# ckonst/VNDecorrelate

Hardware: AMD Instinct MI355X
Metric: Msamples/sec decorrelated (stereo, 30 taps) + achieved HBM GB/s vs roofline (higher is better)
Workload: dtype f32

## Files before the change

### vndecorrelate_amd/csrc/vnd_hooks.hpp

```cpp
#pragma once

extern "C" {

vnd_status vnd_time_convolve_f32_dev(vnd_ctx *ctx, const vnd_taps *t, const float *x, float *y, int64_t batch,
                                     int64_t n, int32_t C, int32_t mode, int32_t n_buffers, int64_t stride,
                                     int32_t iters, void *stream_, float *avg_ms)
{
    vnd_status st = check_shape(ctx, t, batch, n, C, mode);
    if (st != VND_OK) return st;
    if (!avg_ms || iters <= 0 || n_buffers <= 0) return fail(VND_ERR_INVALID, "bad timing arguments");
    DeviceScope on(ctx->device);
    hipStream_t stream = (hipStream_t)stream_;
    hipEvent_t e0 = nullptr, e1 = nullptr;
    hipError_t he = hipEventCreate(&e0);
    if (he == hipSuccess) he = hipEventCreate(&e1);
    if (he == hipSuccess) he = hipEventRecord(e0, stream);
    for (int i = 0; he == hipSuccess && st == VND_OK && i < iters; ++i) {
        const int64_t off = (int64_t)(i % n_buffers) * stride;
        st = launch(ctx, t, x + off, y + off, batch, n, C, mode, stream);
    }
    float ms = 0.f;
    if (he == hipSuccess) he = hipEventRecord(e1, stream);
    if (he == hipSuccess) he = hipEventSynchronize(e1);
    if (he == hipSuccess) he = hipEventElapsedTime(&ms, e0, e1);
// ... 93 lines not shown

vnd_status vnd_spec_kernel_source(int32_t C, const int32_t *tap_offsets, const int32_t *tap_index,
                                  const float *tap_weight, int32_t mode, char *text, int64_t capacity, int64_t *bytes)
{
    if (mode != VND_MODE_FAST && mode != VND_MODE_EXACT)
        return fail(VND_ERR_INVALID, "the specialised kernel exists for VND_MODE_FAST and VND_MODE_EXACT");
    if (!bytes) return fail(VND_ERR_INVALID, "null bytes pointer");
    const Tuning tun = tuning_snapshot();
    SpecTable t;
    if (vnd_status st = spec_table_from_csr(C, tap_offsets, tap_index, tap_weight, nullptr, nullptr, nullptr, 0, &t); st != VND_OK) return st;
    SpecConfig cfg;
    if (!spec_pick_config(t, tun, 160 * 1024, 0, 0, &cfg, false, false, mode == VND_MODE_EXACT)) return fail(VND_ERR_UNSUPPORTED, "halo does not fit the LDS ring");
    cfg.exact = mode == VND_MODE_EXACT ? 1 : 0;
    return source_out(spec_prologue(t, cfg) + kSpecKernelSource, text, capacity, bytes);
}

vnd_status vnd_window_kernel_source(int32_t C, const int32_t *tap_offsets, const int32_t *tap_index,
                                    const float *tap_weight, const int32_t *seg_offsets, const int32_t *seg_end,
                                    const float *seg_gain, int32_t apply_gain, int32_t mode, int32_t frames_per_lane,
                                    int32_t threads, char *text, int64_t capacity, int64_t *bytes,
                                    int64_t *lds_bytes_per_tile, int64_t *fmas_per_tile)
{
    if (mode != VND_MODE_FAST && mode != VND_MODE_EXACT)
        return fail(VND_ERR_INVALID, "the specialised kernel exists for VND_MODE_FAST and VND_MODE_EXACT");
    if (!bytes) return fail(VND_ERR_INVALID, "null bytes pointer");
    const Tuning tun = tuning_snapshot();
    SpecTable t;
    if (vnd_status st = spec_table_from_csr(C, tap_offsets, tap_index, tap_weight, seg_offsets, seg_end, seg_gain, apply_gain, &t); st != VND_OK)
        return st;
    const int M = frames_per_lane, G = tun.win_g > 0 ? tun.win_g : 8;
    WinGeom g;
    bool quad = C % 8 == 0 && tun.win_quad != 0 && tun.win_octet != 0 && win_geometry(t, M, threads, G, false, 160 * 1024, &g, 2);
    quad = quad || ((C % 4 == 0 || (C % 4 == 2 && C >= 6)) && tun.win_quad != 0 && win_geometry(t, M, threads, G, false, 160 * 1024, &g, 1));
    const bool split = !quad && C == 2 && tun.win_split > 0 && win_geometry(t, M, threads, G, false, 160 * 1024, &g, 0, true);
    const bool bc = C == 2 && tun.win_source_fanout != 0;
    if (bc && !win_geometry(t, M, threads, G, true, 160 * 1024, &g, 0, split))
        return fail(VND_ERR_UNSUPPORTED, "this window geometry does not fit the LDS");
    if (!bc && !quad && !split && !win_geometry(t, M, threads, G, false, 160 * 1024, &g))
        return fail(VND_ERR_UNSUPPORTED, "this window geometry does not fit the LDS");
    SpecConfig cfg = win_config(t, g, tun, mode == VND_MODE_EXACT, bc);
    cfg.epi = (tun.win_source_epi != 0 && !bc && !split && (C == 2 || quad)) ? 1 : 0;
    if (lds_bytes_per_tile || fmas_per_tile) {
        size_t lb = 0, fm = 0;
        if (cfg.exact) win_traffic_exact(t, M, &lb, &fm);
        else win_traffic(t, M, &lb, &fm);
        if (lds_bytes_per_tile) *lds_bytes_per_tile = (int64_t)lb;
        if (fmas_per_tile) *fmas_per_tile = (int64_t)fm;
    }
    return source_out(win_source(t, g, cfg), text, capacity, bytes);
}

vnd_status vnd_code_object_private_bytes(const void *code, int64_t bytes, const char *kernel, int64_t *private_bytes)
{
    if (!code || bytes <= 0 || !kernel || !private_bytes) return fail(VND_ERR_INVALID, "bad arguments");
    const std::vector<char> image((const char *)code, (const char *)code + bytes);
    *private_bytes = spec_private_bytes(image, kernel);
    return VND_OK;
}

vnd_status vnd_tuning_read(const char *name, int32_t fallback, int32_t *value)
{
    if (!name || !value) return fail(VND_ERR_INVALID, "null name or value pointer");
    for (const TuningName &v : kTuningNames)
        if (strcmp(v.name, name) == 0) { *value = tuning_value(v, fallback); return VND_OK; }
    *value = fallback;
    return fail(VND_ERR_INVALID, "'%.64s' is not a registered tuning variable (kTuningNames, csrc/vnd_spec.hpp)", name);
}

vnd_status vnd_set_variant(vnd_ctx *ctx, int32_t variant)
// ... 125 lines not shown
```

### vndecorrelate_amd/csrc/vnd_spec.hpp

```cpp
#pragma once
#include <hip/hip_runtime.h>
#include <hip/hiprtc.h>
#include <stdint.h>

#include <sys/stat.h>
#include <sys/types.h>
#include <unistd.h>

#include <algorithm>
#include <cstdarg>
#include <cstring>
#include <cstdio>
#include <cstdlib>
#include <map>
#include <mutex>
#include <string>
#include <tuple>
#include <vector>

namespace vnd {

static const char kSpecKernelSource[] =
#include "vnd_spec_kernel.inc"
    ;

struct SpecConfig {
    int nt = 256;
    int rr = 2;
    int pp = 4;
    int dd = 1;
    int la = 8;
    int nt_stores = 0;
    int exact = 0;
    int epi = 0;
    int bc = 0;
    int shift = 0;
    int win = 0, win_g = 0, win_lds = 0, win_per_cu = 0;
    int win_xpose = 0;
    int win_q = 0;
    int win_s = 0;
    int adds = 0;
    int win_merged = 0;
    int win_late = 0;
    int win_stamps = 0, win_stamp_phases = 0, win_stamp_wave = 0;
    int tile() const { return win ? (win_s ? nt / 2 : (win_q ? nt / (4 * win_q) : nt)) * win : 2 * nt * rr; }
    size_t lds_bytes() const
    {
        if (win) return (size_t)win_lds;
        const size_t pl = (size_t)pp * tile() + 2 * nt + (shift ? 2 : 0);
        return (bc ? 1 : 2) * (shift ? 2 : 1) * pl * 4 + (size_t)2 * (nt / 64) * rr * 2 * 4;
    }
    bool operator<(const SpecConfig &o) const
    {
        return std::tie(nt, rr, pp, dd, la, nt_stores, exact, epi, bc, shift, win, win_g, win_xpose, win_q, win_s, adds, win_merged, win_late,
                        win_stamps, win_stamp_phases, win_stamp_wave) <
               std::tie(o.nt, o.rr, o.pp, o.dd, o.la, o.nt_stores, o.exact, o.epi, o.bc, o.shift, o.win, o.win_g, o.win_xpose, o.win_q, o.win_s,
                        o.adds, o.win_merged, o.win_late, o.win_stamps, o.win_stamp_phases, o.win_stamp_wave);
    }
};

struct SpecTable {
    int C = 0;
    std::vector<int32_t> tap_off;
    std::vector<int32_t> idx;
    std::vector<float> w;
    int max_index = 0;
    std::vector<float> w_raw;
    bool has_seg = false, apply_gain = false;
    std::vector<int32_t> seg_off, seg_end;
    std::vector<float> seg_gain;
};

#define VND_TUNING_VARIABLES(X) \
     \
    X("VND_SPEC_NT", spec_nt, 0) X("VND_SPEC_RR", spec_rr, -1) X("VND_SPEC_DD", spec_dd, -1) X("VND_SPEC_LA", spec_la, -1) \
    X("VND_SPEC_SHIFT", spec_shift, 1) X("VND_WIN_M", win_m, 32) X("VND_WIN_G", win_g, 0) X("VND_WIN_QUAD_M", win_quad_m, 32) \
    X("VND_WIN_SPLIT_LATE", win_split_late, -1) X("VND_WIN_SPLIT_SMALL_NT", win_split_small_nt, 256) \
     \
    X("VND_WIN_EXACT", win_exact, 1) X("VND_WIN_SPLIT_CLASS", win_split_class, 1) X("VND_WIN_QUAD", win_quad, 1) \
    X("VND_WIN_OCTET", win_octet, 1) X("VND_WIN_WIDE", win_wide, 0) X("VND_WIN_SPLIT", win_split, -1) \
    X("VND_WIN_SPLIT_FANOUT", win_split_fanout, 1) X("VND_WIN_FANOUT_EPI", win_fanout_epi, 1) X("VND_WIN_XPOSE_PAIRS", win_xpose_pairs, 1) \
    X("VND_WIN_ADDS", win_adds, 1) X("VND_WIN_EXACT_MERGED", win_exact_merged, 1) \
    X("VND_WIN_SOURCE_FANOUT", win_source_fanout, 0) X("VND_WIN_SOURCE_EPI", win_source_epi, 0) \
    X("VND_EPI_BLOCK_SUMS", epi_block_sums, 1) X("VND_EPI_SUMS_ONLY", epi_sums_only, 1) X("VND_EPI_WIDE", epi_wide, 1) \
    X("VND_EPI_SEQ_SPLIT", epi_seq_split, 1) X("VND_EPI_PAR_COALESCED", epi_par_coalesced, 1) \
     \
    X("VND_WIN_CHUNKS", win_chunks, 1) X("VND_WIN_BALANCE", win_balance, 1) X("VND_WIN_CHUNK_LEN0", win_chunk_len0, 0) \
    X("VND_WIN_STAGGER_TICKS", win_stagger_ticks, 300) X("VND_WIN_PACE", win_pace, 1) X("VND_WIN_PACE_MIN_TILES", win_pace_min_tiles, 16) \
    X("VND_NT_MIN_MB", nt_min_mb, 64) X("VND_NO_NT", no_nt, 0) X("VND_FORCE_NT", force_nt, 0) \
     \
    X("VND_WIN_STAMPS", win_stamps, 0) X("VND_WIN_STAMP_PHASES", win_stamp_phases, 1) X("VND_WIN_STAMP_WAVE", win_stamp_wave, 0)

struct Tuning {
#define VND_TUNING_FIELD(name, field, fallback) int field = fallback;
    VND_TUNING_VARIABLES(VND_TUNING_FIELD)
#undef VND_TUNING_FIELD
};

struct TuningName { const char *name; int Tuning::*field; };
static const TuningName kTuningNames[] = {
#define VND_TUNING_NAME(name, field, fallback) {name, &Tuning::field},
    VND_TUNING_VARIABLES(VND_TUNING_NAME)
#undef VND_TUNING_NAME
};

inline bool spec_tuning()
{
    static const bool on = [] { const char *e = getenv("VND_TUNING"); return e && *e && *e != '0'; }();
    return on;
}
// ... 474 lines not shown
```

### vndecorrelate_amd/csrc/vnd_win.hpp

```cpp
#pragma once
#include "vnd_spec.hpp"
#include <cmath>
#include <functional>

namespace vnd {

static const char kWinKernelSource[] =
#include "vnd_win_kernel.inc"
    ;

struct WinGeom {
    int M = 0, nt = 0, G = 8;
    int C = 2;
    int DE = 0;
    int R = 0;
    int NB = 0;
    int plane = 0;
    int npl = 2;
    int tail = 0;
    int quad = 0;
    int split = 0;
    int nh() const { return split ? nt / 2 : (quad ? nt / (4 * quad) : nt); }
    int quad_pad() const { return quad == 2 ? 16 : 0; }
    size_t lds_bytes() const { return (size_t)(quad ? 2 * quad : 1) * (size_t)npl * (size_t)(M / 4) * (size_t)plane + (size_t)quad_pad(); }
    int tile() const { return nh() * M; }
};

inline int win_workgroups_per_cu(const WinGeom &g);

inline bool win_geometry(const SpecTable &t, int M, int nt, int G, bool bc, size_t lds_limit, WinGeom *g, int quad = 0, bool split = false)
{
    if (split && (t.C != 2 || quad || nt % 128 != 0)) return false;
    if (!(M == 16 || M == 32 || M == 64) || nt % 64 != 0 || nt < 64 || nt > 1024 || G < 1) return false;
    if (quad && (quad > 2 || (t.C % (4 * quad) != 0 && !(quad == 1 && t.C % 4 == 2 && t.C >= 6)) || bc || nt % (256 * quad) != 0 || M * quad > 64 || M > 32)) return false;
    if ((int64_t)t.idx.size() * M > 32768) return false;
    if (t.C < 2 || (t.C & 1) || (bc && t.C != 2)) return false;
    g->M = M; g->nt = nt; g->G = G; g->npl = 2; g->C = t.C; g->quad = quad; g->split = split ? 1 : 0;
    const int nh = g->nh();
    const int qc = M / 4;
    auto lay_out = [&](int de, int tail = 0) {
        g->DE = de;
        g->R = nh + g->DE - tail;
        g->tail = tail;
        g->NB = g->DE / G + 1;
        int units = g->R + G + tail;
        const bool swz = qc == 8;
        const int mod_rule = swz ? 4 : std::max(2, 16 / qc), res_rule = swz ? 2 : std::max(1, 8 / qc);
        while (units % mod_rule != res_rule) ++units;
        g->plane = units * 16;
        if ((size_t)(qc - 1) * g->plane + (size_t)G * 16 >= 65536) return false;
        if ((size_t)qc * g->plane >= 65536) return false;
        return g->lds_bytes() <= lds_limit;
    };
    const int de = (t.max_index + M - 1) / M;
    if (!lay_out(de)) return false;
    const int aligned = de + (16 - (nh + de) % 16) % 16;
    if (aligned != de) {
        const int before = win_workgroups_per_cu(*g);
        WinGeom plain = *g;
        if (!(lay_out(aligned) && win_workgroups_per_cu(*g) >= before)) {
            *g = plain;
            const int cut = (nh + de) % 16;
            if (quad && cut > 0 && nh + de - cut >= nh + G && cut <= (nt / 64) * (64 / (M * quad))) {
                if (!(lay_out(de, cut) && win_workgroups_per_cu(*g) >= before)) *g = plain;
            }
        }
    }
    return true;
}

inline int win_waves_per_simd_max(int M, bool split = false) { return split ? (M <= 32 ? 3 : 2) : (M <= 16 ? 3 : (M <= 32 ? 2 : 1)); }

inline int win_workgroups_per_cu(const WinGeom &g)
{
    const int by_lds = (int)std::min<size_t>(std::min<size_t>(16, 2048 / g.nt), (160 * 1024) / g.lds_bytes());
    const int by_regs = std::max(1, win_waves_per_simd_max(g.M, g.split != 0) * 4 / (g.nt / 64));
    return std::max(1, std::min(by_lds, by_regs));
}

struct WinOp { int kind, acc, half; float w; int tap; };
struct WinRead { int ch, o; std::vector<WinOp> ops; };

inline std::vector<WinRead> win_schedule(const SpecTable &t, int ch, int M)
{
    std::vector<std::pair<int, float>> taps;
    for (int32_t k = t.tap_off[ch]; k < t.tap_off[ch + 1]; ++k)
        if (t.w[k] != 0.0f) taps.push_back({t.idx[k], t.w[k]});
    std::stable_sort(taps.begin(), taps.end(), [](const std::pair<int, float> &a, const std::pair<int, float> &b) { return a.first < b.first; });
    std::vector<WinRead> out;
    if (taps.empty()) return out;
    const int o_last = ((taps.back().first + M - 1) / 4) * 4;
    for (int o = 0; o <= o_last; o += 4) {
        WinRead rd{ch, o, {}};
        for (const auto &tp : taps) {
            const int i = tp.first;
            for (int h = 0; h < 2; ++h) {
                const int j = o + 2 * h - i;
                if ((i & 1) == 0) {
// ... 12 lines not shown

inline void win_traffic(const SpecTable &t, int M, size_t *lds_bytes, size_t *fmas)
{
    *lds_bytes = 0; *fmas = 0;
    for (int ch = 0; ch < t.C; ++ch) {
        *lds_bytes += 16 * win_schedule(t, ch, M).size();
        for (int32_t k = t.tap_off[ch]; k < t.tap_off[ch + 1]; ++k) if (t.w[k] != 0.0f) *fmas += (size_t)M;
    }
}

inline std::string win_taps_name(int pg) { return pg == 0 ? std::string("vw_taps") : "vw_taps_" + std::to_string(pg); }

inline std::string win_taps_channel_name(int pg, int ch)
{
    return pg == 0 ? "vw_taps_c" + std::to_string(ch) : "vw_taps_" + std::to_string(pg) + "c" + std::to_string(ch);
}

inline std::string win_taps_dispatch(const SpecTable &t)
{
    std::string s = "template <int PG> __device__ __forceinline__ void vw_taps_of(vw_lchar *const (&b)[2][VW_NBT], float (&o0)[VW_M], float (&o1)[VW_M])\n{\n";
    for (int pg = 0; pg < t.C / 2; ++pg)
        spec_append(s, "    %sif constexpr (PG == %d) %s(b, o0, o1);\n", pg ? "else " : "", pg, win_taps_name(pg).c_str());
    s += "}\n#define VW_DISPATCH(pg) switch (pg) {";
    for (int pg = 0; pg < t.C / 2; ++pg) spec_append(s, " case %d: vw_span<%d>(a, lds, stream, t_first, ntiles, flags, pace); break;", pg, pg);
    s += " default: break; }\n";
    return s;
}

inline std::string win_rd(const WinGeom &g, int ch, int o)
{
    const int dE = o / g.M, rr = (o % g.M) / 4;
    const int first_tail = g.R - g.nh() + 1;
    char buf[96];
    if (g.tail > 0 && dE >= first_tail) snprintf(buf, sizeof buf, "VW_RD(b[%d][%d], %d)", ch, g.NB + (dE - first_tail), rr * g.plane);
    else { const int kb = dE / g.G; snprintf(buf, sizeof buf, "VW_RD(b[%d][%d], %d)", ch, kb, (dE - kb * g.G) * 16 + rr * g.plane); }
    return buf;
}

inline bool win_adds_ok(const SpecTable &t)
{
    std::vector<float> mags;
    for (size_t k = 0; k < t.w.size(); ++k) {
        const float m = std::fabs(t.w[k]);
        if (m == 0.0f) continue;
        if (!std::isfinite(m) || m < 1e-18f || m > 1e18f) return false;
        if (std::find(mags.begin(), mags.end(), m) == mags.end()) mags.push_back(m);
        if (mags.size() > 8) return false;
    }
    for (int ch = 0; ch < t.C; ++ch) {
        std::vector<std::pair<int, float>> taps;
        for (int32_t k = t.tap_off[ch]; k < t.tap_off[ch + 1]; ++k)
            if (t.w[k] != 0.0f) taps.push_back({t.idx[k], std::fabs(t.w[k])});
        std::stable_sort(taps.begin(), taps.end(), [](const std::pair<int, float> &a, const std::pair<int, float> &b) { return a.first < b.first; });
        int changes = 0;
        for (size_t k = 1; k < taps.size(); ++k) changes += taps[k].second != taps[k - 1].second;
        if (changes > 8) return false;
    }
    return !mags.empty();
}

inline float win_unit_ratio(float from, float to) { return (float)((double)from / (double)to); }

inline void win_emit_adds_op(std::string &s, const std::string &acc, const std::string &x, bool pair, float w, float *unit)
{
    const float mag = std::fabs(w);
    const char sign = std::signbit(w) ? '-' : '+';
    if (*unit == 0.0f) spec_append(s, "    %s = %s %c %s;\n", acc.c_str(), pair ? "Z2" : "0.0f", sign, x.c_str());
// ... 517 lines not shown
        src += "template <int QD> __device__ __forceinline__ void vw_taps_of_channel(int pc, vw_lchar *const (&b)[2][VW_NBT], float (&o)[VW_M])\n{\n";
        const int nq = (t.C + nch - 1) / nch;
        for (int qd = 0; qd < nq; ++qd) {
            const int pair0 = (t.C % nch != 0 && qd == nq - 1) ? (t.C - nch) / 2 : qd * nch / 2;
            spec_append(src, "    %sif constexpr (QD == %d) {\n        switch (pc) {\n", qd ? "else " : "", qd);
            for (int pc = 0; pc < nch; ++pc)
                spec_append(src, "        %s %s(b, o, o); break;\n", pc + 1 < nch ? ("case " + std::to_string(pc) + ":").c_str() : "default:",
                            win_taps_channel_name(pair0 + pc / 2, pc & 1).c_str());
            src += "        }\n    }\n";
        }
        src += "}\n#define VW_TAPS_OF_CHANNEL(pc) vw_taps_of_channel<QD>(pc, b, o);\n#define VW_DISPATCH(pg) switch (pg) {";
        for (int qd = 0; qd < nq; ++qd) spec_append(src, " case %d: vw_span_qc<%d>(a, lds, stream, t_first, ntiles, flags, pace); break;", qd, qd);
        src += " default: break; }\n";
    } else if (g.split) {
        for (int ch = 0; ch < 2; ++ch) src += c.exact ? win_taps_function_exact(t, g, c.la, 0, ch) : win_taps_function(t, g, c.la, 0, ch, c.adds != 0);
        src += "template <int PG> __device__ void vw_taps_of(vw_lchar *const (&b)[2][VW_NBT], float (&o0)[VW_M], float (&o1)[VW_M]);      // (vw_span: not instantiated)\n";
        src += "#define VW_DISPATCH(pg) vw_span_s(a, lds, stream, t_first, ntiles, flags, pace);\n";
    } else {
        const bool merged = c.bc && !c.exact;
        for (int pg = 0; pg < t.C / 2; ++pg) src += c.exact ? (c.win_merged ? win_taps_function_exact_merged(t, g, c.la, pg) : win_taps_function_exact(t, g, c.la, pg)) : (merged ? win_taps_function_merged(t, g, c.la, pg, c.adds != 0) : win_taps_function(t, g, c.la, pg, -1, c.adds != 0));
        src += win_taps_dispatch(t);
    }
    src += fixed.substr(at + marker.size());
    return src;
}

inline SpecConfig win_config(const SpecTable &t, const WinGeom &g, const Tuning &tun, bool exact, bool bc)
{
    SpecConfig c;
    const int M = g.M;
    const bool split = g.split != 0, quad = g.quad != 0;
    c.nt = g.nt; c.win = M; c.win_g = g.G; c.win_lds = (int)g.lds_bytes(); c.win_q = g.quad; c.win_s = g.split;
    c.win_per_cu = win_workgroups_per_cu(g);
    c.rr = 0; c.pp = 0; c.dd = 0;
    c.exact = exact ? 1 : 0; c.bc = bc ? 1 : 0;
    c.la = tun.spec_la >= 0 ? tun.spec_la : ((split && M >= 64) ? (exact ? 3 : 2) : (M >= 32 ? 4 : 6));
    c.win_xpose = (split || quad) ? 0 : (tun.win_xpose_pairs != 0 ? 1 : 0);
    c.adds = (!exact && tun.win_adds != 0 && win_adds_ok(t)) ? 1 : 0;
    c.win_merged = (bc && exact && !split && !quad && tun.win_exact_merged != 0 && win_exact_merged_ok(t)) ? 1 : 0;
    if (split) {
        const int late = M >= 64 ? ((exact && !t.has_seg) ? M / 8 : M / 4 - 1) : 0;
        c.win_late = std::min(std::max(tun.win_split_late >= 0 ? tun.win_split_late : late, 0), M / 4 - 1);
    }
    c.win_stamps = std::min(std::max(tun.win_stamps, 0), 4096);
    c.win_stamp_phases = tun.win_stamp_phases != 0 ? 1 : 0;
    c.win_stamp_wave = std::max(0, tun.win_stamp_wave);
    return c;
}

inline bool win_pick_config(const SpecTable &t, const Tuning &tun, size_t lds_limit, int M, bool small_tiles, bool bc, SpecConfig *out,
                            const std::function<bool(const SpecConfig &)> &rejected, int quad, bool split, bool exact)
{
    static const int kShapes[] = {512, 384, 256, 192, 128, 64};
    const int nt_env = tun.spec_nt, g_env = tun.win_g;
    int best_waves = 0;
    for (int k = 0; k < 6; ++k) {
        const int nt = nt_env > 0 ? nt_env : kShapes[k];
        if (nt_env <= 0 && nt > 256 && quad < 2 && !split) continue;
        if (nt_env <= 0 && nt == 384) continue;
        if (small_tiles && nt_env <= 0 && nt > (quad ? 256 * quad : (split ? tun.win_split_small_nt : 128))) continue;
        for (int G : {8, 4}) {
            if (g_env > 0) G = g_env;
            WinGeom g;
            if (win_geometry(t, M, nt, G, bc, lds_limit, &g, quad, split)) {
                const int waves = win_workgroups_per_cu(g) * (nt / 64);
                if (waves > best_waves) {
                    SpecConfig c = win_config(t, g, tun, exact, bc);
                    if (rejected && rejected(c)) {
                        if (!c.win_xpose) {
                            bool found = false;
                            if (split && M >= 64 && tun.spec_la < 0)
                                while (!found && c.la > 1) { c.la -= 1; found = !rejected(c); }
                            if (!found) continue;
                            best_waves = waves;
                            *out = c;
                            continue;
                        }
                        bool found = false;
                        if (c.la > 3 && tun.spec_la < 0) {
                            c.la -= 1;
                            found = !rejected(c);
                            if (!found) c.la += 1;
                        }
                        if (!found) {
                            c.win_xpose = 0;
                            if (rejected(c)) continue;
                        }
                    }
                    best_waves = waves;
                    *out = c;
                }
            }
            if (g_env > 0) break;
        }
        if (nt_env > 0) break;
    }
    return best_waves > 0;
}

inline std::string win_source_for(const SpecTable &t, const SpecConfig &cfg)
{
    WinGeom g;
    if (!win_geometry(t, cfg.win, cfg.nt, cfg.win_g, cfg.bc != 0, 160 * 1024, &g, cfg.win_q, cfg.win_s != 0)) return "#error window geometry does not fit\n";
    if ((int)g.lds_bytes() != cfg.win_lds) return "#error window geometry changed between the launch plan and the build\n";
    return win_source(t, g, cfg);
}

}
```

### vndecorrelate_amd/csrc/vnd_win_kernel.inc

```
R"VNDWIN(
// vnd_spec_kernel, WINDOW form - the per-table tap sum with a register window (gfx950, wave64).
//
// Compiled at run time with hipRTC (vnd_win.hpp) behind a generated prologue that defines
//   VW_NT   threads per workgroup                 VW_M   consecutive output frames a lane owns per tile (16 | 32 | 64)
//   VW_R    ring entries (one entry = the M frames of one lane's run): NT of the tile + VW_DE of halo
//   VW_G    entries mirrored behind the ring, = the reach of one base register
//   VW_NB   base registers per channel (VW_DE / VW_G + 1)
//   VW_PLANE  bytes between the LDS planes of consecutive 16-byte chunks of an entry
//   VW_LA   LDS reads kept in flight ahead of the FMAs
//   VW_C    interleaved channels of the signal (even): a workgroup takes ONE channel pair of a span, 8 bytes of
//           every VW_C*4-byte frame (VW_C = 2: the whole frame, 16-byte accesses)
//   VW_Q    1: the QUAD form for signals of 4k channels - a workgroup takes a channel QUAD of a span (16 bytes of every
//           frame), a wave computes ONE channel of it (tap functions vw_taps_<pair>c<channel>) and stages and stores whole
//           16-byte pieces for all four (vw_span_qc below)
//           2: the OCTET form for signals of 8k channels - two neighbouring quads (32 bytes of every frame: with 8 channels,
//           whole frames and whole cache lines) per workgroup, an eighth of its lanes per channel
//   VW_S    1: the SPLIT form of a stereo signal - half the workgroup's waves compute channel 0, the others channel 1 (the tap
//           functions vw_taps_c0 / vw_taps_c1): a lane carries one channel's accumulators, so three waves fit a SIMD's registers
//           where the plain form holds two (vw_span_s below)
// and the functions vw_taps(), vw_taps_1(), ... (at the marker below): the tap sum of ONE lane for each channel
// pair, fully unrolled, with vw_taps_of<PG>() to pick one and VW_DISPATCH(pg): the span loop vw_span<pg> of a run-time pair number.
//
// The reference's tap sum (decorrelation.py:649-658, :402-414) asks, per output sample, for one input sample
// per tap.  vnd_spec_kernel.inc reads each of them from LDS (one aligned ds_read_b64 per tap and output
// ... 62 lines not shown
    int epi_nblocks;
    int epi_rows_major;      // 1: [stream][block][x0 x1 y0 y1] instead - the rows epilogue_reduce_kernel adds up (the fused fast stage)
    // PACING of a CU's two co-resident workgroups (one round of persistent workgroups): the SIMDs issue the OLDER wave first, so the
    // workgroup publishes its count of finished tiles in its CU's slot pair and reads its partner's: the one BEHIND runs its next tile at
    // raised wave priority.  pace: [CU index][2] counters in device memory (never reset: a stale count only costs the first tile its bias)
    unsigned *pace;
};

struct VWPace { unsigned *mine; const unsigned *other; unsigned done; };

constexpr int VW_NW = VW_NT / 64;
constexpr int VW_QC = VW_M / 4;                 // 16-byte chunks per entry and channel
constexpr int VW_NH = VW_S ? VW_NT / 2 : VW_Q ? VW_NT / (4 * VW_Q) : VW_NT;  // lanes - and ring entries of a tile - per channel pair
constexpr int VW_T = VW_NH * VW_M;              // frames per tile
constexpr int VW_LPE = VW_Q ? VW_M * VW_Q : VW_M / 2;  // lanes of a 1 KB global access that fall into one entry (a lane moves a frame pair; VW_Q: one frame of four channels)
constexpr int VW_EPI_N = 64 / VW_LPE;           // entries per 1 KB global access
constexpr int VW_NI = VW_M / 2;                 // 1 KB global accesses per wave and tile
constexpr int VW_NPL = 2;                       // plane sets in LDS: one per output channel (the store phase transposes both channels' runs through them)
constexpr int VW_NXP = (VW_BC && !VW_S) ? 1 : 2; // ... of them holding INPUT: a mono input is staged once for both outputs (in the split form into both sets)
constexpr int VW_CH = VW_QC * VW_PLANE;         // byte offset of channel 1's planes
constexpr int VW_CX = VW_BC ? 1 : VW_C;         // interleaved INPUT channels
// channel pairs (VW_Q: quads or octets): one per workgroup and span.  4k + 2 channels (6, 10, ...) as QUADS: k full quads and one more that
// starts at channel C - 4 - it overlaps its neighbour in one channel pair, which both workgroups compute and write with the same bits
// (a frame's 16 bytes per access instead of the pair form's 8, for (k + 1) / (k + 1/2) of the arithmetic)
constexpr int VW_PAIRS = VW_Q ? (VW_C + 4 * VW_Q - 1) / (4 * VW_Q) : VW_C / 2;
constexpr int VW_PAIRB = 2 * VW_CH;             // VW_Q: byte offset of the second pair's plane sets
constexpr int VW_QUADB = 2 * VW_PAIRB + VW_QUADPAD; // octets: ... of the second QUAD's (shifted by 16 bytes: the two quads of a frame - neighbouring lanes of the 4-byte staging accesses - in different banks)
static_assert(VW_C >= 2 && VW_C % 2 == 0 && (VW_C == 2 || !VW_BC) && (VW_C == 2 || VW_Q || !VW_EPI), "whole channel pairs; fan-out and fused pointwise steps are stereo (quads / octets: the normaliser's sums only)");
static_assert(VW_Q == 0 || VW_Q == 1 || VW_Q == 2, "pairs, quads or octets");
static_assert(!VW_S || (VW_C == 2 && !VW_Q && !VW_EPI && VW_NT % 128 == 0 && VW_M >= 16), "split form: a stereo table, whole waves per channel");
static_assert(!VW_Q || ((VW_C % (4 * VW_Q) == 0 || (VW_Q == 1 && VW_C % 4 == 2 && VW_C >= 6)) && VW_NT % (256 * VW_Q) == 0 && VW_M * VW_Q <= 64 && VW_M <= 32), "quad / octet form: whole channel quads (4k + 2 channels: the last quad overlaps), whole waves per channel");
static_assert(VW_M == 16 || VW_M == 32 || VW_M == 64, "run length");
constexpr int VW_NBT = VW_NB + VW_TAIL;          // base registers per channel: the ring's, then one per entry offset that reaches into the tail
static_assert(VW_NT % 64 == 0 && VW_R >= VW_NH && VW_R + VW_TAIL == VW_NH + VW_DE && (VW_TAIL == 0 || (VW_Q && VW_R % 16 == 0)), "ring (+ tail) = tile + halo");
static_assert(VW_NB * VW_G > VW_DE, "bases cover the halo");
static_assert((VW_PLANE / 16) >= VW_R + VW_G + VW_TAIL, "plane stride: room for ring + mirror (+ tail)");
static_assert((VW_QC - 1) * VW_PLANE + VW_G * 16 < 65536 && VW_CH < 65536, "ds offset field is 16 bits");
static_assert((VW_Q ? 2 * VW_Q : 1) * VW_NPL * VW_QC * VW_PLANE + VW_QUADPAD <= 160 * 1024 && VW_QUADPAD % 16 == 0, "LDS");

// Raw buffer descriptor (stride 0): num_records = bytes left in the stream, so loads past the end of
// the stream return 0 (the reference's dropped terms, decorrelation.py:656-658) and stores past it
// are discarded.  Built from kernel arguments, blockIdx and the tile counter only: lives in SGPRs.
__device__ __forceinline__ v4i vw_rsrc(const void *base, long long bytes)
{
    const long long cap = 0x7fffffff;
    const unsigned long long addr = (unsigned long long)base;
    v4i r;
    r.x = (int)(unsigned)addr;
    r.y = (int)((unsigned)(addr >> 32) & 0xffffu);
    r.z = (int)(bytes < 0 ? 0 : (bytes > cap ? cap : bytes));
    r.w = 0x00020000;
    return r;
}

// blocks b and b + 8 share an XCD (and its L2): give one XCD consecutive logical ids, so that neighbouring
// spans (whose halos overlap) share an L2
__device__ __forceinline__ unsigned vw_xcd_remap(unsigned b, unsigned nwg)
{
    const unsigned q = nwg >> 3, r = nwg & 7u, xcd = b & 7u;
    const unsigned start = xcd < r ? xcd * (q + 1) : r * (q + 1) + (xcd - r) * q;
    return start + (b >> 3);
}

// (a mod R) for a < 2R, without a comparison: a - R wraps past 2^32 when a < R
__device__ __forceinline__ unsigned vw_wrap(unsigned a)
{
    const unsigned b = a - (unsigned)VW_R;
// ... 563 lines not shown
}
#endif

#if VW_S
// ---- the SPLIT form of a stereo signal: a wave computes ONE channel ---------------------------------------
// The plain form's lane carries both channels' work one after the other: E / P accumulators, the first channel's finished
// outputs and a tile of prefetched frames - ~240 registers, two waves per SIMD.  Here waves 0 .. NW/2-1 run channel 0's tap
// function (vw_taps_c0) on the tile's NT/2 entries and the other half channel 1's: per lane one channel's accumulators, half
// the prefetch - three waves per SIMD fit (two workgroups of 384 lanes per CU: 12 waves), on the same ring and the same
// 1 KB global accesses.  A frame's two channels now sit in two waves: outputs go as planar runs into the tile's dead
// entries, one barrier more, then each wave reads back and stores the 32 entries it also refills (as vw_span_qc).
template <int CH>
__device__ __forceinline__ void vw_taps_ch(vw_lchar *const (&b)[2][VW_NBT], float (&o)[VW_M])
{
    if constexpr (CH == 0) vw_taps_c0(b, o, o);
    else vw_taps_c1(b, o, o);
}

__device__ __forceinline__ void vw_span_s(const VWArgs &a, vw_lchar *lds, long long stream, int t_first, int ntiles, int flags, VWPace &pace)
{
    constexpr int NWH = VW_NW / 2;                                       // waves per channel
    constexpr int NI = VW_M / 4;                                         // 1 KB global STORES per wave and tile (64 frame pairs each)
    // VW_BC - a mono input fanned out: the one input channel is staged into BOTH plane sets (each output channel's waves read their own
    // copy with the tap functions of the stereo form unchanged), 16 bytes = 4 frames per lane and access: half as many input accesses,
    // each 256 frames = 256 / M ring entries (stereo: 128 frames)
    constexpr int NIN = VW_BC ? VW_M / 8 : VW_M / 4;                     // 1 KB global LOADS per wave and tile
    constexpr int EIN = VW_BC ? 256 / VW_M : VW_EPI_N;                   // ring entries per load
    constexpr int XB = VW_BC ? 4 : 8;                                    // input bytes per frame
    // the refill's frames: NE accesses are prefetched a tile ahead and held in registers through the tap phase, the other
    // LATE are loaded at the start of the store phase that consumes them (64-frame runs: the accumulators need the room)
    constexpr int LATE = VW_LATE < NIN ? VW_LATE : NIN - 1;
    constexpr int NE = NIN - LATE;
    static_assert(VW_LATE >= 0 && LATE < NIN, "late refill accesses");
    const int tid = threadIdx.x;
    const int ln = tid & 63;
    const int wv = __builtin_amdgcn_readfirstlane(tid >> 6);
    const int pc = wv >= NWH ? 1 : 0;                                    // the wave's channel
    const int wl = wv - pc * NWH;
    const int tl = wl * 64 + ln;                                         // the entry of a tile this LANE computes (in its channel)
    const int we = wl * 64 + pc * 32;                                    // the first of the 32 entries this WAVE stages and stores (both channels)
    const long long f0 = (long long)t_first * VW_T;
    const float *xs = a.x + (stream * a.n + f0) * (XB / 4);
    float *ys = a.y + (stream * a.n + f0) * 2;
    const long long bytes_left = (a.n - f0) * 8;                         // (of the output)
    const long long need = ((long long)ntiles * VW_T + (long long)VW_DE * VW_M) * XB;
    const long long bytes_need = need < (a.n - f0) * XB ? need : (a.n - f0) * XB;
#if VW_LANE_SWIZZLE
    const int lq = (ln & ~24) | ((ln & 8) << 1) | ((ln & 16) >> 1);      // (as vw_span: the 8-byte staging writes and read-backs touch every bank once)
#else
    const int lq = ln;
#endif
    const int lane_e = lq / VW_LPE;
    const int lane_at = ((lq % VW_LPE) >> 1) * VW_PLANE + (lq & 1) * 8;
    // ... and in a 1 KB LOAD: stereo as above; mono - 4 frames = one 16-byte chunk of entry ln / (M / 4), written to both plane sets
    const int in_e = VW_BC ? ln / (VW_M / 4) : lane_e;
    const int in_at = VW_BC ? (ln % (VW_M / 4)) * VW_PLANE : lane_at;
    const int in16 = VW_BC ? ln * 16 : lq * 16;                          // the lane's byte offset in a load
    auto stage = [&](vw_lchar *at, v4f v) {
        if constexpr (VW_BC) { *(vw_lv4f *)at = v; *(vw_lv4f *)(at + VW_CH) = v; }
        else vw_write_pair(at, v);
    };
#if VW_STAMPS && VW_STAMP_PHASES
    const bool vw_stamp_on = blockIdx.x < VW_STAMPS && (a.chunk_tiles > 0 || a.bal_total > 0 || (unsigned)(stream * a.spans + t_first / a.tiles_per_span) == vw_xcd_remap(blockIdx.x, a.nblocks));
    if (vw_stamp_on && threadIdx.x == 0) {
        unsigned hw, xcc;
        asm volatile("s_getreg_b32 %0, hwreg(HW_REG_HW_ID)" : "=s"(hw));
        asm volatile("s_getreg_b32 %0, hwreg(HW_REG_XCC_ID)" : "=s"(xcc));
        vw_stamps[blockIdx.x * 16 + 15] = (unsigned long long)hw | ((unsigned long long)xcc << 32);
    }
#endif
    VW_STAMP_DECL;
    VW_STAMP(0);

    {
        const v4i rx = vw_rsrc(xs, bytes_need);
        constexpr int NFILL = (VW_R + EIN - 1) / EIN;
        constexpr int PER = (NFILL + VW_NW - 1) / VW_NW;
        constexpr int BATCH = 8;
        for (int k0 = 0; k0 < PER; k0 += BATCH) {
            v4f w[BATCH];
#pragma unroll
            for (int kk = 0; kk < BATCH; ++kk) {
                const int i = wv + VW_NW * (k0 + kk);
                w[kk] = vw_load4(rx, i * 1024 + in16, 0, VW_LOAD_AUX);
            }
#pragma unroll
            for (int kk = 0; kk < BATCH; ++kk) {
                const int i = wv + VW_NW * (k0 + kk);
                const int e = i * EIN + in_e;
                if (k0 + kk < PER && e < VW_R) {
                    stage(lds + in_at + e * 16, w[kk]);
                    if (e < VW_G) stage(lds + in_at + (e + VW_R) * 16, w[kk]);
                }
            }
        }
    }
    v4f pre[NE];
    {
        const long long f = ((long long)VW_R + we) * VW_M;
        const v4i rx = vw_rsrc(xs + f * (XB / 4), bytes_need - f * XB);
#pragma unroll
        for (int m = 0; m < NE; ++m) pre[m] = vw_load4(rx, 1024 * m + in16, 0, VW_LOAD_AUX);
    }
    asm volatile("s_waitcnt lgkmcnt(0)\n\ts_barrier" ::: "memory");
    VW_STAMP(1);
    bool hi = (flags & 2) != 0;                                          // (wave-uniform) raised priority: a chunk's first workgroup - or, paced, the one behind
    if (hi) __builtin_amdgcn_s_setprio(2);

    unsigned p0 = 0;
    for (int t = 0; t < ntiles; ++t) {
        // the last tile of the workgroup's last unit refills nothing: no loads, no staging writes, no barrier behind its stores
        const bool fin = (flags & 1) != 0 && t == ntiles - 1;
        const unsigned pw = vw_wrap(p0 + (unsigned)we);
        const unsigned pl = vw_wrap(p0 + (unsigned)tl);
        // (a lane's byte offset in a 1 KB access and its entry in it, made opaque per tile: hipcc otherwise hoists the sums with
        //  64-frame runs is what spilled)
        int lq16 = lq * 16, in16o = in16;
        unsigned pwl = pw + (unsigned)lane_e, pwi = pw + (unsigned)in_e;
        asm volatile("" : "+v"(lq16), "+v"(pwl));
        if constexpr (VW_BC) asm volatile("" : "+v"(in16o), "+v"(pwi));
        float o[VW_M];
        {
            vw_lchar *b[2][VW_NBT];
#pragma unroll
            for (int k = 0; k < VW_NB; ++k) {
                b[0][k] = lds + vw_wrap(pl + (unsigned)(k * VW_G)) * 16u;
                b[1][k] = b[0][k] + VW_CH;
            }
            if (pc == 0) vw_taps_ch<0>(b, o);
            else vw_taps_ch<1>(b, o);
        }
#pragma unroll
        for (int j = 0; j < VW_M; ++j) asm volatile("" : "+v"(o[j]));
        VW_STAMP_TILE(t, 0);
        // X. every wave is done reading this tile's window: the tile's own entries are dead (both channels)
        asm volatile("s_waitcnt lgkmcnt(0)\n\ts_barrier" ::: "memory");
        VW_STAMP_TILE(t, 1);
        if (hi) __builtin_amdgcn_s_setprio(3);
        else __builtin_amdgcn_s_setprio(1);
        // (pacing: the partner's count, in flight through the store phase)
        unsigned seen = 0;
        if (pace.other != nullptr) seen = __hip_atomic_load(pace.other, __ATOMIC_RELAXED, __HIP_MEMORY_SCOPE_AGENT);
        // (the late part of THIS tile's refill: in flight through the transposition and the stores)
        v4f late[LATE > 0 ? LATE : 1];
        if constexpr (LATE > 0) {                                        // (also on a final tile: out of range there, no data moves)
            const long long fl = ((long long)t * VW_NH + VW_R + we) * VW_M;
            const v4i rl = vw_rsrc(xs + fl * (XB / 4), bytes_need - fl * XB);
#pragma unroll
            for (int m = 0; m < LATE; ++m) late[m] = vw_load4(rl, (VW_BC ? in16o : lq16) + 1024 * (NE + m), 0, VW_LOAD_AUX);
        }
        // the lane's run into its own dead entry, planar (its channel's planes)
        vw_lchar *const mine = lds + pc * VW_CH + pl * 16u;
#pragma unroll
        for (int r = 0; r < VW_QC; ++r)
            *(vw_lv4f *)(mine + r * VW_PLANE) = v4f{o[4 * r], o[4 * r + 1], o[4 * r + 2], o[4 * r + 3]};
        // X2. ... and the partner wave's (the other channel of the same 64 entries)
        asm volatile("s_waitcnt lgkmcnt(0)\n\ts_barrier" ::: "memory");
        VW_STAMP_TILE(t, 2);
        const long long fo = (long long)t * VW_T + (long long)we * VW_M;
        const v4i ry = vw_rsrc(ys + fo * 2, bytes_left - fo * 8);
        const long long fi = ((long long)(t + 1) * VW_NH + VW_R + we) * VW_M;
        const v4i rx = vw_rsrc(xs + fi * (XB / 4), bytes_need - fi * XB);
        constexpr int ST_AUX = VW_NT_STORES ? VW_NT_STORE_AUX : 0;
        //  short launch nothing much, covers these round trips: tools/ablate/RUNS.md: run_r4c, run_r4g.sh)
#pragma unroll
        for (int m = 0; m < NI; ++m) {
            vw_lchar *at = lds + lane_at + vw_wrap(pwl + (unsigned)(m * VW_EPI_N)) * 16u;
            const v2f r0 = *(const volatile vw_lv2f *)at, r1 = *(const volatile vw_lv2f *)(at + VW_CH);
            vw_store4(v4f{r0.x, r1.x, r0.y, r1.y}, ry, lq16 + 1024 * m, 0, ST_AUX);
        }
        if (!fin) {
            const bool mirror = pw < (unsigned)VW_G || pw + 32u > (unsigned)VW_R;             // wave-uniform
#pragma unroll
            for (int m = 0; m < NIN; ++m) {
                const unsigned e = vw_wrap((VW_BC ? pwi : pwl) + (unsigned)(m * EIN));
                vw_lchar *at = lds + in_at + e * 16u;
                const v4f v = m < NE ? pre[m < NE ? m : 0] : late[m >= NE ? m - NE : 0];
                stage(at, v);
                if (mirror) { if (e < (unsigned)VW_G) stage(at + VW_R * 16, v); }
                if (m < NE) pre[m < NE ? m : 0] = vw_load4(rx, (VW_BC ? in16o : lq16) + 1024 * m, 0, VW_LOAD_AUX);
            }
        }
        p0 = p0 + VW_NH >= VW_R ? p0 + VW_NH - VW_R : p0 + VW_NH;
        pace.done += 1;
        if (pace.other != nullptr) {
            if (threadIdx.x == 0) __hip_atomic_store(pace.mine, pace.done, __ATOMIC_RELAXED, __HIP_MEMORY_SCOPE_AGENT);
            hi = (unsigned)__builtin_amdgcn_readfirstlane((int)seen) > pace.done;       // the partner is ahead: this workgroup's next tile goes first
        }
        if (hi) __builtin_amdgcn_s_setprio(2);
        else __builtin_amdgcn_s_setprio(0);
        // Y. the refill is in place for every wave's window
        if (!fin) asm volatile("s_waitcnt lgkmcnt(0)\n\ts_barrier" ::: "memory");
        VW_STAMP_TILE(t, 3);
    }
    if (hi) __builtin_amdgcn_s_setprio(0);
    VW_STAMP_FLUSH(vw_stamp_on);
}
#endif

// VW_WAVES_PER_EU: the waves per SIMD that the LDS footprint and the registers let a CU hold - as minimum AND maximum:
// the scheduler must not trade registers for an occupancy the LDS will not grant
extern "C" __global__ __launch_bounds__(VW_NT) __attribute__((amdgpu_waves_per_eu(VW_WAVES_PER_EU, VW_WAVES_PER_EU)))
void vnd_spec_kernel(const VWArgs a)
{
#if VW_STAMPS
    { const unsigned long long entry_ = __builtin_amdgcn_s_memrealtime(); if (threadIdx.x == 0 && blockIdx.x < VW_STAMPS) vw_stamps[blockIdx.x * 16 + 12] = entry_; }
#endif
    extern __shared__ __attribute__((aligned(16))) float lds_generic[];
    vw_lchar *lds = (vw_lchar *)(vw_lfloat *)lds_generic;
    // One round of workgroups: more units than resident slots are walked inside the kernel
    // (the channel pairs of a span are neighbouring units: their workgroups touch the same lines at about the same time)
    const unsigned first = vw_xcd_remap(blockIdx.x, a.nblocks);
    // (ONE call site of the span loop - it is the whole tap sum, inlined - for both ways of cutting the work)
// ... 67 lines not shown
```

Measured before the change: 669,700.

## Cut the stereo split-window ring to a multiple of 16 with a tail behind the mirror

Extends the ring-plus-tail window layout, previously used only by the quad form, to the stereo split kernel at run length 64. The ring is cut to a multiple of 16 entries and the last halo entries move to a tail slot behind the mirror. Wave 0 swaps old and new tail entries during each refill, and tap reads pick ring or tail bases per lane. The layout is kept only if it needs no more LDS and no fewer workgroups per CU, so the aim is better occupancy or LDS use. It costs extra selects, swaps and indexing complexity in wave 0's refill path.

```diff
diff --git a/vndecorrelate_amd/csrc/vnd_hooks.hpp b/vndecorrelate_amd/csrc/vnd_hooks.hpp
--- a/vndecorrelate_amd/csrc/vnd_hooks.hpp
+++ b/vndecorrelate_amd/csrc/vnd_hooks.hpp
@@ -149,9 +149,9 @@
     WinGeom g;
     bool quad = C % 8 == 0 && tun.win_quad != 0 && tun.win_octet != 0 && win_geometry(t, M, threads, G, false, 160 * 1024, &g, 2);
     quad = quad || ((C % 4 == 0 || (C % 4 == 2 && C >= 6)) && tun.win_quad != 0 && win_geometry(t, M, threads, G, false, 160 * 1024, &g, 1));
-    const bool split = !quad && C == 2 && tun.win_split > 0 && win_geometry(t, M, threads, G, false, 160 * 1024, &g, 0, true);
+    const bool split = !quad && C == 2 && tun.win_split > 0 && win_geometry(t, M, threads, G, false, 160 * 1024, &g, 0, true, tun.win_cut_stereo != 0);
     const bool bc = C == 2 && tun.win_source_fanout != 0;
-    if (bc && !win_geometry(t, M, threads, G, true, 160 * 1024, &g, 0, split))
+    if (bc && !win_geometry(t, M, threads, G, true, 160 * 1024, &g, 0, split, tun.win_cut_stereo != 0))
         return fail(VND_ERR_UNSUPPORTED, "this window geometry does not fit the LDS");
     if (!bc && !quad && !split && !win_geometry(t, M, threads, G, false, 160 * 1024, &g))
         return fail(VND_ERR_UNSUPPORTED, "this window geometry does not fit the LDS");
diff --git a/vndecorrelate_amd/csrc/vnd_spec.hpp b/vndecorrelate_amd/csrc/vnd_spec.hpp
--- a/vndecorrelate_amd/csrc/vnd_spec.hpp
+++ b/vndecorrelate_amd/csrc/vnd_spec.hpp
@@ -42,6 +42,7 @@
     int adds = 0;
     int win_merged = 0;
     int win_late = 0;
+    int win_cut = 0;
     int win_stamps = 0, win_stamp_phases = 0, win_stamp_wave = 0;
     int tile() const { return win ? (win_s ? nt / 2 : (win_q ? nt / (4 * win_q) : nt)) * win : 2 * nt * rr; }
     size_t lds_bytes() const
@@ -52,10 +53,10 @@
     }
     bool operator<(const SpecConfig &o) const
     {
-        return std::tie(nt, rr, pp, dd, la, nt_stores, exact, epi, bc, shift, win, win_g, win_xpose, win_q, win_s, adds, win_merged, win_late,
+        return std::tie(nt, rr, pp, dd, la, nt_stores, exact, epi, bc, shift, win, win_g, win_xpose, win_q, win_s, adds, win_merged, win_late, win_cut,
                         win_stamps, win_stamp_phases, win_stamp_wave) <
                std::tie(o.nt, o.rr, o.pp, o.dd, o.la, o.nt_stores, o.exact, o.epi, o.bc, o.shift, o.win, o.win_g, o.win_xpose, o.win_q, o.win_s,
-                        o.adds, o.win_merged, o.win_late, o.win_stamps, o.win_stamp_phases, o.win_stamp_wave);
+                        o.adds, o.win_merged, o.win_late, o.win_cut, o.win_stamps, o.win_stamp_phases, o.win_stamp_wave);
     }
 };
 
@@ -75,7 +76,7 @@
      \
     X("VND_SPEC_NT", spec_nt, 0) X("VND_SPEC_RR", spec_rr, -1) X("VND_SPEC_DD", spec_dd, -1) X("VND_SPEC_LA", spec_la, -1) \
     X("VND_SPEC_SHIFT", spec_shift, 1) X("VND_WIN_M", win_m, 32) X("VND_WIN_G", win_g, 0) X("VND_WIN_QUAD_M", win_quad_m, 32) \
-    X("VND_WIN_SPLIT_LATE", win_split_late, -1) X("VND_WIN_SPLIT_SMALL_NT", win_split_small_nt, 256) \
+    X("VND_WIN_SPLIT_LATE", win_split_late, -1) X("VND_WIN_SPLIT_SMALL_NT", win_split_small_nt, 256) X("VND_WIN_CUT_STEREO", win_cut_stereo, 1) \
      \
     X("VND_WIN_EXACT", win_exact, 1) X("VND_WIN_SPLIT_CLASS", win_split_class, 1) X("VND_WIN_QUAD", win_quad, 1) \
     X("VND_WIN_OCTET", win_octet, 1) X("VND_WIN_WIDE", win_wide, 0) X("VND_WIN_SPLIT", win_split, -1) \
diff --git a/vndecorrelate_amd/csrc/vnd_win.hpp b/vndecorrelate_amd/csrc/vnd_win.hpp
--- a/vndecorrelate_amd/csrc/vnd_win.hpp
+++ b/vndecorrelate_amd/csrc/vnd_win.hpp
@@ -28,7 +28,7 @@
 
 inline int win_workgroups_per_cu(const WinGeom &g);
 
-inline bool win_geometry(const SpecTable &t, int M, int nt, int G, bool bc, size_t lds_limit, WinGeom *g, int quad = 0, bool split = false)
+inline bool win_geometry(const SpecTable &t, int M, int nt, int G, bool bc, size_t lds_limit, WinGeom *g, int quad = 0, bool split = false, bool cut_stereo = true)
 {
     if (split && (t.C != 2 || quad || nt % 128 != 0)) return false;
     if (!(M == 16 || M == 32 || M == 64) || nt % 64 != 0 || nt < 64 || nt > 1024 || G < 1) return false;
@@ -64,6 +64,9 @@
             if (quad && cut > 0 && nh + de - cut >= nh + G && cut <= (nt / 64) * (64 / (M * quad))) {
                 if (!(lay_out(de, cut) && win_workgroups_per_cu(*g) >= before)) *g = plain;
             }
+            if (split && M == 64 && cut_stereo && cut > 0 && nh + de - cut >= nh + G) {
+                if (!(lay_out(de, cut) && win_workgroups_per_cu(*g) >= before && g->lds_bytes() <= plain.lds_bytes())) *g = plain;
+            }
         }
     }
     return true;
@@ -142,7 +145,8 @@
     const int dE = o / g.M, rr = (o % g.M) / 4;
     const int first_tail = g.R - g.nh() + 1;
     char buf[96];
-    if (g.tail > 0 && dE >= first_tail) snprintf(buf, sizeof buf, "VW_RD(b[%d][%d], %d)", ch, g.NB + (dE - first_tail), rr * g.plane);
+    if (g.tail > 0 && dE >= first_tail && g.split) snprintf(buf, sizeof buf, "VW_RD(b[%d][%d], %d)", ch, g.NB + (dE - first_tail), (dE - (dE / g.G) * g.G) * 16 + rr * g.plane);
+    else if (g.tail > 0 && dE >= first_tail) snprintf(buf, sizeof buf, "VW_RD(b[%d][%d], %d)", ch, g.NB + (dE - first_tail), rr * g.plane);
     else { const int kb = dE / g.G; snprintf(buf, sizeof buf, "VW_RD(b[%d][%d], %d)", ch, kb, (dE - kb * g.G) * 16 + rr * g.plane); }
     return buf;
 }
@@ -726,6 +730,7 @@
     const bool split = g.split != 0, quad = g.quad != 0;
     c.nt = g.nt; c.win = M; c.win_g = g.G; c.win_lds = (int)g.lds_bytes(); c.win_q = g.quad; c.win_s = g.split;
     c.win_per_cu = win_workgroups_per_cu(g);
+    c.win_cut = (split && g.tail > 0) ? 1 : 0;
     c.rr = 0; c.pp = 0; c.dd = 0;
     c.exact = exact ? 1 : 0; c.bc = bc ? 1 : 0;
     c.la = tun.spec_la >= 0 ? tun.spec_la : ((split && M >= 64) ? (exact ? 3 : 2) : (M >= 32 ? 4 : 6));
@@ -756,7 +761,7 @@
         for (int G : {8, 4}) {
             if (g_env > 0) G = g_env;
             WinGeom g;
-            if (win_geometry(t, M, nt, G, bc, lds_limit, &g, quad, split)) {
+            if (win_geometry(t, M, nt, G, bc, lds_limit, &g, quad, split, tun.win_cut_stereo != 0)) {
                 const int waves = win_workgroups_per_cu(g) * (nt / 64);
                 if (waves > best_waves) {
                     SpecConfig c = win_config(t, g, tun, exact, bc);
@@ -795,7 +800,7 @@
 inline std::string win_source_for(const SpecTable &t, const SpecConfig &cfg)
 {
     WinGeom g;
-    if (!win_geometry(t, cfg.win, cfg.nt, cfg.win_g, cfg.bc != 0, 160 * 1024, &g, cfg.win_q, cfg.win_s != 0)) return "#error window geometry does not fit\n";
+    if (!win_geometry(t, cfg.win, cfg.nt, cfg.win_g, cfg.bc != 0, 160 * 1024, &g, cfg.win_q, cfg.win_s != 0, cfg.win_cut != 0)) return "#error window geometry does not fit\n";
     if ((int)g.lds_bytes() != cfg.win_lds) return "#error window geometry changed between the launch plan and the build\n";
     return win_source(t, g, cfg);
 }
diff --git a/vndecorrelate_amd/csrc/vnd_win_kernel.inc b/vndecorrelate_amd/csrc/vnd_win_kernel.inc
--- a/vndecorrelate_amd/csrc/vnd_win_kernel.inc
+++ b/vndecorrelate_amd/csrc/vnd_win_kernel.inc
@@ -118,7 +118,7 @@
 static_assert(!VW_Q || ((VW_C % (4 * VW_Q) == 0 || (VW_Q == 1 && VW_C % 4 == 2 && VW_C >= 6)) && VW_NT % (256 * VW_Q) == 0 && VW_M * VW_Q <= 64 && VW_M <= 32), "quad / octet form: whole channel quads (4k + 2 channels: the last quad overlaps), whole waves per channel");
 static_assert(VW_M == 16 || VW_M == 32 || VW_M == 64, "run length");
 constexpr int VW_NBT = VW_NB + VW_TAIL;          // base registers per channel: the ring's, then one per entry offset that reaches into the tail
-static_assert(VW_NT % 64 == 0 && VW_R >= VW_NH && VW_R + VW_TAIL == VW_NH + VW_DE && (VW_TAIL == 0 || (VW_Q && VW_R % 16 == 0)), "ring (+ tail) = tile + halo");
+static_assert(VW_NT % 64 == 0 && VW_R >= VW_NH && VW_R + VW_TAIL == VW_NH + VW_DE && (VW_TAIL == 0 || ((VW_Q || (VW_S && VW_M == 64)) && VW_R % 16 == 0)), "ring (+ tail) = tile + halo");
 static_assert(VW_NB * VW_G > VW_DE, "bases cover the halo");
 static_assert((VW_PLANE / 16) >= VW_R + VW_G + VW_TAIL, "plane stride: room for ring + mirror (+ tail)");
 static_assert((VW_QC - 1) * VW_PLANE + VW_G * 16 < 65536 && VW_CH < 65536, "ds offset field is 16 bits");
@@ -748,6 +748,16 @@
     constexpr int LATE = VW_LATE < NIN ? VW_LATE : NIN - 1;
     constexpr int NE = NIN - LATE;
     static_assert(VW_LATE >= 0 && LATE < NIN, "late refill accesses");
+    // The TAIL (VW_TAIL > 0: the ring cut to a multiple of 16 entries, win_geometry): the window's last VW_TAIL entries live behind the
+    // mirror.  A tile's refill stays the one contiguous run of NH entries it was: the ring's dead entries 0 .. TAIL-1 of the tile take
+    // the OLD tail (moved inside LDS), entries TAIL .. NH-1 the run's first NH - TAIL entries, and the run's last TAIL entries are the
+    // NEW tail.  All of that falls to the wave that owns the tile's first 32 entries (wave 0): in its first NTM accesses the lanes of
+    // entries < TAIL load the entry NH further on (TSH bytes), swap it with the old tail's in LDS - a read and a write of the same
+    // address by the same lane, in program order - and stage what they read where the load would have gone.  Every other access of
+    // every wave is what it was: the refill stays wave-private, barrier Y publishes ring and tail together.
+    constexpr int NTM = (VW_TAIL + EIN - 1) / EIN;                       // accesses (of wave 0) that hold tail entries
+    constexpr int TSH = VW_NH * VW_M * XB;                               // bytes from an entry of the old tail to the same entry of the next
+    static_assert(VW_TAIL < 32 && TSH + 1024 * NIN < (1 << 20), "the tail inside the first wave's entries");
     const int tid = threadIdx.x;
     const int ln = tid & 63;
     const int wv = __builtin_amdgcn_readfirstlane(tid >> 6);
@@ -790,7 +800,7 @@
 
     {
         const v4i rx = vw_rsrc(xs, bytes_need);
-        constexpr int NFILL = (VW_R + EIN - 1) / EIN;
+        constexpr int NFILL = (VW_R + VW_TAIL + EIN - 1) / EIN;      // (the tail's entries follow the ring's in the stream)
         constexpr int PER = (NFILL + VW_NW - 1) / VW_NW;
         constexpr int BATCH = 8;
         for (int k0 = 0; k0 < PER; k0 += BATCH) {
@@ -804,8 +814,8 @@
             for (int kk = 0; kk < BATCH; ++kk) {
                 const int i = wv + VW_NW * (k0 + kk);
                 const int e = i * EIN + in_e;
-                if (k0 + kk < PER && e < VW_R) {
-                    stage(lds + in_at + e * 16, w[kk]);
+                if (k0 + kk < PER && e < VW_R + VW_TAIL) {
+                    stage(lds + in_at + (e < VW_R ? e : e + VW_G) * 16, w[kk]);      // ring slot e, or tail slot behind the mirror
                     if (e < VW_G) stage(lds + in_at + (e + VW_R) * 16, w[kk]);
                 }
             }
@@ -816,7 +826,7 @@
         const long long f = ((long long)VW_R + we) * VW_M;
         const v4i rx = vw_rsrc(xs + f * (XB / 4), bytes_need - f * XB);
 #pragma unroll
-        for (int m = 0; m < NE; ++m) pre[m] = vw_load4(rx, 1024 * m + in16, 0, VW_LOAD_AUX);
+        for (int m = 0; m < NE; ++m) pre[m] = vw_load4(rx, 1024 * m + in16 + ((m < NTM && wv == 0 && m * EIN + in_e < VW_TAIL) ? TSH : 0), 0, VW_LOAD_AUX);
     }
     asm volatile("s_waitcnt lgkmcnt(0)\n\ts_barrier" ::: "memory");
     VW_STAMP(1);
@@ -835,6 +845,13 @@
         unsigned pwl = pw + (unsigned)lane_e, pwi = pw + (unsigned)in_e;
         asm volatile("" : "+v"(lq16), "+v"(pwl));
         if constexpr (VW_BC) asm volatile("" : "+v"(in16o), "+v"(pwi));
+        // (wave 0's lanes of tail entries load TSH bytes further on; the lane's entry of the access from the opaque sums: nothing new is held)
+        const unsigned ine = (VW_BC ? pwi : pwl) - pw;
+        // (an access whose entries are ALL tail entries shifts the whole wave: a scalar)
+        auto tail_sh = [&](int m) -> int {
+            if (m >= NTM || wv != 0) return 0;
+            return ((m + 1) * EIN <= VW_TAIL || (unsigned)(m * EIN) + ine < (unsigned)VW_TAIL) ? TSH : 0;
+        };
         float o[VW_M];
         {
             vw_lchar *b[2][VW_NBT];
@@ -843,6 +860,24 @@
                 b[0][k] = lds + vw_wrap(pl + (unsigned)(k * VW_G)) * 16u;
                 b[1][k] = b[0][k] + VW_CH;
             }
+#if VW_TAIL
+            // entry offsets VW_R - VW_NH + 1 ... VW_DE: in the ring for the tile's first lanes, in the tail for its last ones.  The tap
+            // functions read them at base + (offset - k G) * 16 (k = offset / G) like every other offset, through a base of their own:
+            // the ring's base k for the lanes that find the entry in the ring (or its mirror), the tail's slot of entry offset k G for
+            // the others - one select per offset and tile, its lane mask a loop invariant in scalar registers; the tail's address from
+            // an opaque copy of the lane's entry, so that it is not carried through the tap phases as a loop invariant
+            int tlo = tl;
+            asm volatile("" : "+v"(tlo));
+#pragma unroll
+            for (int j = 0; j < VW_TAIL; ++j) {
+                const unsigned d = (unsigned)(VW_R - VW_NH + 1 + j);
+                const int k = (int)d / VW_G;
+                vw_lchar *const tb = lds + ((unsigned)tlo + (unsigned)(k * VW_G + VW_G)) * 16u;     // slot R + G + (e - R) of e = lane + k G
+                const bool in_tail = (unsigned)tl + d >= (unsigned)VW_R;
+                b[0][VW_NB + j] = in_tail ? tb : b[0][k];
+                b[1][VW_NB + j] = in_tail ? tb + VW_CH : b[1][k];
+            }
+#endif
             if (pc == 0) vw_taps_ch<0>(b, o);
             else vw_taps_ch<1>(b, o);
         }
@@ -863,7 +898,7 @@
             const long long fl = ((long long)t * VW_NH + VW_R + we) * VW_M;
             const v4i rl = vw_rsrc(xs + fl * (XB / 4), bytes_need - fl * XB);
 #pragma unroll
-            for (int m = 0; m < LATE; ++m) late[m] = vw_load4(rl, (VW_BC ? in16o : lq16) + 1024 * (NE + m), 0, VW_LOAD_AUX);
+            for (int m = 0; m < LATE; ++m) late[m] = vw_load4(rl, (VW_BC ? in16o : lq16) + 1024 * (NE + m) + tail_sh(NE + m), 0, VW_LOAD_AUX);
         }
         // the lane's run into its own dead entry, planar (its channel's planes)
         vw_lchar *const mine = lds + pc * VW_CH + pl * 16u;
@@ -887,14 +922,49 @@
         }
         if (!fin) {
             const bool mirror = pw < (unsigned)VW_G || pw + 32u > (unsigned)VW_R;             // wave-uniform
-#pragma unroll
-            for (int m = 0; m < NIN; ++m) {
+            // one access of the refill into its ring entries; `swap`: the lanes of tail entries put what they loaded (the NEXT tail's
+            // entry) into the tail's slot and the old tail's entry `keep` - read from that slot before - into the ring
+            auto refill = [&](int m, bool swap, v4f keep) {
                 const unsigned e = vw_wrap((VW_BC ? pwi : pwl) + (unsigned)(m * EIN));
                 vw_lchar *at = lds + in_at + e * 16u;
-                const v4f v = m < NE ? pre[m < NE ? m : 0] : late[m >= NE ? m - NE : 0];
+                v4f v = m < NE ? pre[m < NE ? m : 0] : late[m >= NE ? m - NE : 0];
+                if (swap) {
+                    const unsigned i = (unsigned)(m * EIN) + ine;
+                    if ((m + 1) * EIN <= VW_TAIL || i < (unsigned)VW_TAIL) {
+                        stage(lds + in_at + ((unsigned)(VW_R + VW_G) + i) * 16u, v);
+                        v = keep;
+                    }
+                }
                 stage(at, v);
                 if (mirror) { if (e < (unsigned)VW_G) stage(at + VW_R * 16, v); }
-                if (m < NE) pre[m < NE ? m : 0] = vw_load4(rx, (VW_BC ? in16o : lq16) + 1024 * m, 0, VW_LOAD_AUX);
+                if (m < NE) pre[m < NE ? m : 0] = vw_load4(rx, (VW_BC ? in16o : lq16) + 1024 * m + tail_sh(m), 0, VW_LOAD_AUX);
+            };
+            if constexpr (VW_TAIL > 0) {
+                // the accesses that hold tail entries (0 .. NTM-1, wave 0's) ride between the others: the old tail's entry is read from
+                // its slot GAP accesses before it is needed - one in flight at a time, four registers, no wait
+                constexpr int GAP = NIN - NTM >= 2 * NTM ? 2 : 1;
+                static_assert(NIN - NTM >= NTM * GAP, "the tail's accesses between the others");
+                v4f told = {0.0f, 0.0f, 0.0f, 0.0f};
+#pragma unroll
+                for (int mm = 0; mm < NIN - NTM; ++mm) {
+                    const int j = mm / GAP;                                   // the tail access that rides here
+                    if (j < NTM && mm % GAP == 0 && wv == 0) {              // (wave-uniform)
+                        const unsigned i = (unsigned)(j * EIN) + ine;
+                        if ((j + 1) * EIN <= VW_TAIL || i < (unsigned)VW_TAIL) {
+                            const vw_lchar *ta = lds + in_at + ((unsigned)(VW_R + VW_G) + i) * 16u;
+                            if constexpr (VW_BC) told = *(const volatile vw_lv4f *)ta;
+                            else {
+                                const v2f r0 = *(const volatile vw_lv2f *)ta, r1 = *(const volatile vw_lv2f *)(ta + VW_CH);
+                                told = v4f{r0.x, r1.x, r0.y, r1.y};
+                            }
+                        }
+                    }
+                    refill(NTM + mm, false, told);
+                    if (j < NTM && mm % GAP == GAP - 1) refill(j, wv == 0, told);
+                }
+            } else {
+#pragma unroll
+                for (int m = 0; m < NIN; ++m) refill(m, false, v4f{0.0f, 0.0f, 0.0f, 0.0f});
             }
         }
         p0 = p0 + VW_NH >= VW_R ? p0 + VW_NH - VW_R : p0 + VW_NH;
```

Result: no change. 671,800, median of 5 (+0.3%).
